# marl/l3embedding

Hardware: AMD Instinct MI355X
Metric: AVC training pairs/sec (1s audio + 224x224 frame) (higher is better)
Workload: dtype f32; 1 GPU; full cnn_L3_melspec2 AVC training step (audio+vision+fusion, fwd+bwd+Adam), batch 64 per GPU, global batch 64, fp32, inputs resident in HBM; global_batch=64, parallelism=dp1, fp32_conv=f4x4

## Files before the change

include/l3hip.h:

```cpp
#ifndef L3HIP_H
#define L3HIP_H

#include <stdint.h>

#ifdef __cplusplus
extern "C" {
#endif

#define L3_OK 0
#define L3_EINVAL (-1)
#define L3_EHIP (-2)
#define L3_ENOMEM (-3)
#define L3_ESTATE (-4)
#define L3_ECOMM (-5)

#define L3_MODEL_CNN_L3_ORIG 0
#define L3_MODEL_TINY_L3 1
#define L3_MODEL_CNN_L3_KAPREDBINPUTBN 2
#define L3_MODEL_CNN_L3_MELSPEC1 3
#define L3_MODEL_CNN_L3_MELSPEC2 4

typedef struct l3_engine l3_engine;

#define L3_DTYPE_F32 0
// ... 125 lines not shown
int l3_op_conv2d_fwd(int device, const float *x, const float *w, const float *b, float *y,
                     int n, int h, int wd, int cin, int cout, int kh, int kw, int same);
int l3_op_conv2d_bwd(int device, const float *x, const float *w, const float *dy,
                     float *dx, float *dw, float *db,
                     int n, int h, int wd, int cin, int cout, int kh, int kw, int same);
int l3_op_bn_relu_fwd(int device, const float *x, const float *gamma, const float *beta,
                      float *y, float *mean, float *var, int64_t rows, int c, int relu, int x_bf16);
int l3_op_bn_relu_bwd(int device, const float *x, const float *y, const float *dy,
                      const float *gamma, const float *beta, const float *mean, const float *var,
                      float *dx, float *dgamma, float *dbeta, int64_t rows, int c, int relu, int x_bf16);
int l3_op_bn_relu_pool2_fwd(int device, const float *x, const float *gamma, const float *beta, float *p,
                            float *mean, float *var, int n, int h, int wd, int c, int same, int relu_mode, int x_bf16);
int l3_op_bn_relu_pool2_bwd(int device, const float *x, const float *gamma, const float *beta, const float *dp,
                            float *dx, float *dgamma, float *dbeta, float *dbias, int n, int h, int wd, int c,
                            int same, int relu_mode, int x_bf16);
int l3_op_maxpool_fwd(int device, const float *x, float *y, int n, int h, int wd, int c,
                      int ph, int pw, int sh, int sw, int same);
int l3_op_maxpool_bwd(int device, const float *x, const float *dy, float *dx, int n, int h,
                      int wd, int c, int ph, int pw, int sh, int sw, int same);
int l3_op_frontend(int device, int model_type, const float *audio, int n, int db_max_scope, float *out);
int l3_op_gather_frames(int device, const float *samples, int64_t n_samples, const int64_t *table,
                        int64_t n_frames, float *frames);
int l3_op_resample(int device, const float *x, int64_t n_in, int64_t sr_orig, int64_t sr_new, const double *half_window,
                   int64_t n_window, int num_table, int64_t t0, int64_t n_out, float *y);
int l3_op_resample_clips(int device, const float *x, int64_t n_in, const int64_t *clips, int64_t n_clips, int64_t sr_new,
                         const double *half_window, int64_t n_window, int num_table, int64_t n_samples, int copy_equal,
                         float *y);
int l3_op_bn_stats_from_partials(int device, const float *part, int nblk, int c, const float *pivot, int64_t rows,
                                 float eps, float *mean, float *var);
int l3_op_conv2d_fwd_stats(int device, int dtype, const float *x, const float *w, const float *b, float *y, float *part, int *nblk,
// ... 205 lines not shown
```

l3embedding_amd/_lib.py:

```python
import ctypes as C
import os

import numpy as np

from . import _build

MODEL_IDS = {
    'cnn_L3_orig': 0,
    'tiny_L3': 1,
    'cnn_L3_kapredbinputbn': 2,
    'cnn_L3_melspec1': 3,
    'cnn_L3_melspec2': 4,
}

FAMILIES = ('conv_fwd', 'conv_dgrad', 'conv_wgrad', 'elementwise', 'frontend', 'head', 'adam')


DTYPES = {'f32': 0, 'fp32': 0, 'float32': 0, 'bf16': 1}
FP32_CONV = {'f4x4': 0, 'f2x2': 1, 'f2x2_bf16x6': 2}
DP_MOVING = {'replicas': 0, 'rank_local': 1}
OP_DTYPES = dict(DTYPES, bf16_stored=2, bf16_stored_out=3)


class L3Config(C.Structure):
# ... 89 lines not shown
    'l3_sync': (C.c_int, [C.c_void_p]),
    'l3_profile_enable': (C.c_int, [C.c_void_p, C.c_int]),
    'l3_set_tower_overlap': (C.c_int, [C.c_void_p, C.c_int]),
    'l3_profile_read_executed': (C.c_int, [C.c_void_p, C.c_int, C.POINTER(C.c_double)]),
    'l3_profile_read_bytes': (C.c_int, [C.c_void_p, C.c_int, C.POINTER(C.c_double)]),
    'l3_profile_read': (C.c_int, [C.c_void_p, C.c_int, C.POINTER(C.c_double), C.POINTER(C.c_int64),
                                  C.POINTER(C.c_double)]),
    'l3_op_conv2d_fwd': (C.c_int, [C.c_int, C.c_void_p, C.c_void_p, C.c_void_p, C.c_void_p] + [C.c_int] * 8),
    'l3_op_conv2d_fwd_dt': (C.c_int, [C.c_int, C.c_int, C.c_void_p, C.c_void_p, C.c_void_p, C.c_void_p] + [C.c_int] * 8),
    'l3_op_conv2d_bwd_dt': (C.c_int, [C.c_int, C.c_int] + [C.c_void_p] * 6 + [C.c_int] * 8),
    'l3_op_conv2d_bwd': (C.c_int, [C.c_int] + [C.c_void_p] * 6 + [C.c_int] * 8),
    'l3_op_bn_relu_fwd': (C.c_int, [C.c_int] + [C.c_void_p] * 6 + [C.c_int64, C.c_int, C.c_int, C.c_int]),
    'l3_op_bn_relu_bwd': (C.c_int, [C.c_int] + [C.c_void_p] * 10 + [C.c_int64, C.c_int, C.c_int, C.c_int]),
    'l3_op_bn_relu_pool2_fwd': (C.c_int, [C.c_int] + [C.c_void_p] * 6 + [C.c_int] * 7),
    'l3_op_bn_relu_pool2_bwd': (C.c_int, [C.c_int] + [C.c_void_p] * 8 + [C.c_int] * 7),
    'l3_op_maxpool_fwd': (C.c_int, [C.c_int, C.c_void_p, C.c_void_p] + [C.c_int] * 9),
    'l3_op_maxpool_bwd': (C.c_int, [C.c_int, C.c_void_p, C.c_void_p, C.c_void_p] + [C.c_int] * 9),
    'l3_op_frontend': (C.c_int, [C.c_int, C.c_int, C.c_void_p, C.c_int, C.c_int, C.c_void_p]),
    'l3_op_gather_frames': (C.c_int, [C.c_int, C.c_void_p, C.c_int64, C.c_void_p, C.c_int64, C.c_void_p]),
    'l3_op_resample': (C.c_int, [C.c_int, C.c_void_p, C.c_int64, C.c_int64, C.c_int64, C.c_void_p, C.c_int64, C.c_int,
                                 C.c_int64, C.c_int64, C.c_void_p]),
    'l3_op_resample_clips': (C.c_int, [C.c_int, C.c_void_p, C.c_int64, C.c_void_p, C.c_int64, C.c_int64, C.c_void_p, C.c_int64,
                                       C.c_int, C.c_int64, C.c_int, C.c_void_p]),
    'l3_op_bn_stats_from_partials': (C.c_int, [C.c_int, C.c_void_p, C.c_int, C.c_int, C.c_void_p, C.c_int64, C.c_float,
                                               C.c_void_p, C.c_void_p]),
    'l3_op_conv2d_fwd_stats': (C.c_int, [C.c_int, C.c_int] + [C.c_void_p] * 5 + [C.POINTER(C.c_int), C.c_void_p, C.c_void_p] +
                               [C.c_int] * 9),
    'l3_op_conv2d_dgrad_bn_bwd': (C.c_int, [C.c_int, C.c_int] + [C.c_void_p] * 9 + [C.POINTER(C.c_int), C.c_void_p, C.c_void_p] +
                                  [C.c_int] * 9 + [C.c_int64]),
    'l3_op_bn_relu_pool2_fwd_xwin': (C.c_int, [C.c_int] + [C.c_void_p] * 7 + [C.c_int] * 7),
# ... 627 lines not shown
                                      _ptr(var), n, h, wd, c, int(same), int(relu_mode), flags))
    return p, mean, var


def op_bn_relu_pool2_bwd(x, gamma, beta, dp, same, device=0, relu_mode=1, x_bf16=False, out_bf16=False):
    lib = load()
    x, dp = _f32(x), _f32(dp)
    n, h, wd, c = x.shape
    dx = np.empty_like(x)
    dg, db, dbias = (np.empty((c,), np.float32) for _ in range(3))
    check(lib.l3_op_bn_relu_pool2_bwd(device, _ptr(x), _ptr(_f32(gamma)), _ptr(_f32(beta)), _ptr(dp), _ptr(dx),
                                      _ptr(dg), _ptr(db), _ptr(dbias), n, h, wd, c, int(same), int(relu_mode), int(x_bf16) | (4 if out_bf16 else 0)))
    return dx, dg, db, dbias


def _pool_out(h, p, s, same):
    return -(-h // s) if same else (h - p) // s + 1


def op_maxpool_fwd(x, ph, pw, sh, sw, same, device=0):
    lib = load()
    x = _f32(x)
    n, h, wd, c = x.shape
    y = np.empty((n, _pool_out(h, ph, sh, same), _pool_out(wd, pw, sw, same), c), np.float32)
    check(lib.l3_op_maxpool_fwd(device, _ptr(x), _ptr(y), n, h, wd, c, ph, pw, sh, sw, int(same)))
    return y


def op_maxpool_bwd(x, dy, ph, pw, sh, sw, same, device=0):
    lib = load()
# ... 1044 lines not shown
```

l3embedding_amd/csrc/bn_fused.hip:

```cpp
#include "kernels.h"
#include "device_common.h"

namespace l3 {



__device__ __forceinline__ void store_quad(void* base, int64_t q, f32x4 v, int obf) {
    if (obf) {
        bf16x4 h;
        h[0] = (__bf16)v.x; h[1] = (__bf16)v.y; h[2] = (__bf16)v.z; h[3] = (__bf16)v.w;
        __builtin_nontemporal_store(h, reinterpret_cast<bf16x4*>(base) + q);
    } else {
        __builtin_nontemporal_store(v, reinterpret_cast<f32x4*>(base) + q);
    }
}

template <bool XBF>
__device__ __forceinline__ f32x4 load_quad(const void* base, int64_t q) {
    if constexpr (XBF) {
        const u32x2 r = __builtin_nontemporal_load(reinterpret_cast<const u32x2*>(base) + q);
        return f32x4{__uint_as_float(r.x << 16), __uint_as_float(r.x & 0xffff0000u), __uint_as_float(r.y << 16),
                     __uint_as_float(r.y & 0xffff0000u)};
    } else {
        return __builtin_nontemporal_load(reinterpret_cast<const f32x4*>(base) + q);
// ... 563 lines not shown
    const int nb_a = fast_blocks(work_a);
    float* part2 = dbias ? part : nullptr;
    using ApplyFn = void (*)(const void*, const void*, const f32x4*, const f32x4*, const f32x4*, const f32x4*, const f32x4*, void*,
                             float*, int64_t, Pool2Geom, int, int);
    static const ApplyFn apply_fns[8] = {
        bn_bwd_apply_fast_kernel<false, false, false>, bn_bwd_apply_fast_kernel<false, false, true>,
        bn_bwd_apply_fast_kernel<false, true, false>,  bn_bwd_apply_fast_kernel<false, true, true>,
        bn_bwd_apply_fast_kernel<true, false, false>,  bn_bwd_apply_fast_kernel<true, false, true>,
        bn_bwd_apply_fast_kernel<true, true, false>,   bn_bwd_apply_fast_kernel<true, true, true>};
    hipLaunchKernelGGL(apply_fns[variant], dim3(nb_a), dim3(FB), 0, s, xv, dyv, sc4, sh4, reinterpret_cast<const f32x4*>(cA),
                       reinterpret_cast<const f32x4*>(cB), reinterpret_cast<const f32x4*>(cC), (void*)dx, part2, n4, g, relu,
                       dx_bf16);
    if (dbias) launch_fast_final(SumFinal{dbias}, part, nb_a, C, s);
}

}
```

l3embedding_amd/csrc/elementwise.hip:

```cpp
#include <algorithm>

#include "kernels.h"

namespace l3 {

static constexpr int RED_BLOCK = 256;
static constexpr int RED_MAX_BLOCKS = 1024;
static constexpr int SMALLC_MAX = 16;

static inline int red_blocks(int64_t rows, int C) {
    int rows_per_pass = (C % 4 == 0 && C >= 4 && C <= 1024) ? (RED_BLOCK / (C / 4) > 0 ? RED_BLOCK / (C / 4) : 1) : RED_BLOCK;
    int64_t b = (rows + (int64_t)rows_per_pass * 16 - 1) / ((int64_t)rows_per_pass * 16);
    if (b < 1) b = 1;
    if (b > RED_MAX_BLOCKS) b = RED_MAX_BLOCKS;
    return (int)b;
}

size_t colreduce_scratch_floats(int64_t rows, int C) {
    const size_t a = (size_t)red_blocks(rows, C) * 2 * (size_t)(C < 4 ? 4 : C) + 64;
    const size_t b = bn_fast_ok(C) ? bn_fast_scratch_floats(C) : 0;
    return a > b ? a : b;
}

template <class F>
// ... 510 lines not shown
    int arg[4];
    const size_t base = (size_t)n * P * C + cb * 64 + cq * 4;
    gp_scan(x + base, P, C, pg, best, arg);
    gp_merge(sb, sa, pg, cq, best, arg);
    const gp4 d = *reinterpret_cast<const gp4*>(dy + (size_t)n * out_batch_stride + cb * 64 + cq * 4);
    int am[4];
#pragma unroll
    for (int e = 0; e < 4; ++e) am[e] = sa[0][cq * 4 + e];
    for (int p = pg; p < P; p += 16) {
        gp4 o;
#pragma unroll
        for (int e = 0; e < 4; ++e) o[e] = p == am[e] ? d[e] : 0.f;
        *reinterpret_cast<gp4*>(dx + base + (size_t)p * C) = o;
    }
}
static bool is_global_pool(const PoolGeom& g) {
    return g.Ho == 1 && g.Wo == 1 && g.padT == 0 && g.padL == 0 && g.ph == g.H && g.pw == g.W && g.C % 64 == 0 &&
           g.out_batch_stride % 4 == 0;
}

void maxpool_fwd(const float* x, float* y, const PoolGeom& g, hipStream_t s) {
    if (is_global_pool(g)) {
        hipLaunchKernelGGL(global_maxpool_fwd_kernel, dim3(g.N * (g.C / 64)), dim3(256), 0, s, x, y, g.H * g.W, g.C,
                           (int64_t)g.out_batch_stride);
        return;
    }
    const int64_t total = (int64_t)g.N * g.Ho * g.Wo * g.C;
    hipLaunchKernelGGL(maxpool_fwd_kernel, dim3(ew_blocks(total)), dim3(256), 0, s, x, y, g);
}
__global__ __launch_bounds__(256) void maxpool_bwd_kernel(const float* x, const float* dy, float* dx, PoolGeom g) {
    const int64_t total = (int64_t)g.N * g.Ho * g.Wo * g.C;
// ... 395 lines not shown
```

l3embedding_amd/csrc/engine.hip:

```cpp
#include <hip/hip_runtime.h>
#include "knobs.h"

#include <cmath>
#include <cstdio>
#include <cstdlib>
#include <cstring>
#include <map>
#include <string>
#include <vector>

#include "../../include/l3hip.h"
#include "comm.h"
#include "conv_path.h"
#include "kernels.h"

namespace {

using namespace l3;

static thread_local std::string g_create_error;

constexpr float BN_EPS = 1e-3f;
constexpr float BN_MOMENTUM = 0.99f;
constexpr float L2_WEIGHT = 1e-5f;
// ... 28 lines not shown
};

enum FirstWgrad { FW_NONE, FW_AUG, FW_AUG_DEFERRED };
struct ConvPlan {
    ConvStorage st;
    ConvFwdPath fwd;
    int stat_mode = 0;
    FirstWgrad aug = FW_NONE;
    ConvWgradPath wgrad;
    bool colsum = false;
    ConvDgradPath dgrad;
    int bwd_bn = -1;
    double fwd_bytes = 0.0, wg_bytes = 0.0, dg_bytes = 0.0;
};
enum BnStats { BS_PARTIALS, BS_FAST, BS_PLAIN, BS_MOVING };
enum BnBwd { BB_BY_FIRST_CONV, BB_FAST_POOLED, BB_FAST, BB_FAST_DEFERRED, BB_PLAIN };
struct BnPlan {
    BnStats stats = BS_MOVING;
    int stat_blocks = 0;
    BnBwd bwd = BB_PLAIN;
    int bwd_blocks = 0;
    double fwd_bytes = 0.0, bwd_bytes = 0.0;
};

struct Op {
    OpKind kind;
    std::string name;
    int in = 0, out = 0;
    int block = 0, bucket = 0;
    int kh = 0, kw = 0, cout = 0;
    bool same = false;
// ... 6 lines not shown
    bool fused_first = false;
    bool defer_apply = false;
    int bn_defer = -1;
    float *xaug = nullptr, *gaug = nullptr;
    ConvGeom ageom{};
    int bn_follow = -1;
    bool need_dx = true;
    int dy_to_bn = -1;
    float* xwin = nullptr;
    int p_gamma = -1, p_beta = -1, p_mmean = -1, p_mvar = -1;
    bool fused_relu = false;
    bool prerelu = false;
    int fuse_pool = -1;
    int bias_param = -1;
    bool fused_into_bn = false;
    bool bias_by_bn = false;
    float *mean = nullptr, *var = nullptr, *scale = nullptr, *shift = nullptr;
    float *biased_mean = nullptr, *biased_var = nullptr;
    PoolGeom pg{};
    ConvPlan cp{};
    BnPlan bp{};
};

struct Tower {
    std::string prefix;
    std::vector<Tensor> t;
    std::vector<Op> ops;
    int nblocks = 0;
    int emb_conv_op = -1;
    bool training = false;
// ... 464 lines not shown
                    bn.fused_first = true;
                    op.ageom = op.geom;
                    op.ageom.Cin = op.geom.Cin + 1;
                }
                break;
            }
    const int nbv = e->vis.nblocks, nba = e->aud.nblocks;
    for (auto& op : e->vis.ops) op.bucket = 1 + (nbv - 1 - op.block);
    for (auto& op : e->aud.ops) op.bucket = 1 + nbv + (nba - 1 - op.block);
    for (Tower* tw : {&e->vis, &e->aud})
        for (auto& op : tw->ops) {
            for (int pi : {op.p_kernel, op.p_bias, op.p_gamma, op.p_beta})
                if (pi >= 0) e->params[pi].bucket = op.bucket;
        }
    for (int pi : {e->p_w1, e->p_b1, e->p_w2, e->p_b2}) e->params[pi].bucket = 0;
    for (Tower* tw : {&e->vis, &e->aud})
        for (size_t i = 0; i < tw->ops.size(); ++i) {
            Op& op = tw->ops[i];
            if (op.kind != OP_BN || !bn_fast_ok(tw->t[op.in].C)) continue;
            if (i > 0 && tw->ops[i - 1].kind == OP_CONV) {
                op.bias_param = tw->ops[i - 1].p_bias;
                tw->ops[i - 1].bias_by_bn = true;
                tw->ops[i - 1].bn_follow = (int)i;
            }
            const bool pool_next = i + 2 < tw->ops.size() && tw->ops[i + 1].kind == OP_POOL &&
                                   tw->ops[i + 1].pg.ph == 2 && tw->ops[i + 1].pg.pw == 2 && tw->ops[i + 1].pg.sh == 2 &&
                                   tw->ops[i + 1].pg.sw == 2 && tw->ops[i + 1].pg.padT == 0 && tw->ops[i + 1].pg.padL == 0;
            if (op.fused_relu && pool_next) {
                op.fuse_pool = (int)i + 1;
                tw->ops[i + 1].fused_into_bn = true;
            } else if (!op.fused_relu && pool_next && i >= 2 && tw->ops[i - 1].kind == OP_RELU &&
                       tw->ops[i - 2].kind == OP_CONV) {
                op.prerelu = true;
                op.in = tw->ops[i - 2].out;
                tw->ops[i - 1].fused_into_bn = true;
                op.bias_param = tw->ops[i - 2].p_bias;
                tw->ops[i - 2].bias_by_bn = true;
                tw->ops[i - 2].bn_follow = (int)i;
                op.fuse_pool = (int)i + 1;
                tw->ops[i + 1].fused_into_bn = true;
            }
        }
    const int first_wg_fuse = knob_int("L3_FIRST_WG_FUSE", 1);
    if (first_wg_fuse)
        for (Tower* tw : {&e->vis, &e->aud})
            for (auto& cv : tw->ops) {
                if (cv.kind != OP_CONV || cv.in_bn < 0 || cv.bn_follow < 0 || !cv.bias_by_bn) continue;
                Op& bn = tw->ops[cv.bn_follow];
                if (bn.kind == OP_BN && bn.fuse_pool < 0 && !bn.prerelu && bn.in == cv.out && bn_fast_ok(cv.cout) &&
                    conv_first_wgrad_ok(cv.ageom)) {
                    bn.defer_apply = true;
                    cv.bn_defer = cv.bn_follow;
                }
            }
    const int pooled_fuse = knob_int("L3_BNBWD_FUSE_POOLED", 1);
    if (bnbwd_fuse && pooled_fuse)
        for (Tower* tw : {&e->vis, &e->aud})
            for (size_t i = 0; i < tw->ops.size(); ++i) {
                Op& cv = tw->ops[i];
                if (cv.kind != OP_CONV || !cv.need_dx || cv.dy_to_bn >= 0) continue;
                for (size_t j = 0; j < i; ++j) {
                    const Op& bn = tw->ops[j];
                    if (bn.kind == OP_BN && bn.fuse_pool >= 0 && tw->ops[bn.fuse_pool].out == cv.in && (bn.fused_relu != bn.prerelu) &&
                        bn_fast_ok(tw->t[bn.in].C))
// ... 325 lines not shown
        tw.t[0].d = ti == 0 ? e->video : nullptr;
        if (ti == 1) {
            if ((rc = dev_alloc_t(e, &tw.t[0].d, (size_t)tw.t[0].numel()))) return rc;
        }
        const int64_t concat_off = ti == 0 ? 0 : e->nv;
        for (size_t oi = 0; oi < tw.ops.size(); ++oi) {
            Op& op = tw.ops[oi];
            Tensor& y = tw.t[op.out];
            const bool last = oi + 1 == tw.ops.size();
            if (last) {
                y.d = e->h0 + concat_off;
                y.g = e->dh0 + concat_off;
                y.batch_stride = D;
                y.alias = true;
                if (op.kind == OP_POOL) op.pg.out_batch_stride = D;
            } else if ((op.kind == OP_BN && op.fuse_pool >= 0) || (op.kind == OP_RELU && op.fused_into_bn)) {
                if (op.kind == OP_BN) {
                    bool wanted = false;
                    for (size_t ci = 0; ci < tw.ops.size(); ++ci)
                        if (tw.ops[ci].kind == OP_CONV && tw.ops[ci].dy_to_bn == (int)oi) wanted = true;
                    const Tensor& pl = tw.t[tw.ops[op.fuse_pool].out];
                    if (wanted && (rc = dev_alloc_t(e, &op.xwin, t_floats(pl, tw.t[op.in].d_bf16)))) return rc;
                }
            } else {
                if ((rc = dev_alloc_t(e, &y.d, t_floats(y, y.d_bf16)))) return rc;
                if ((rc = dev_alloc_t(e, &y.g, t_floats(y, y.g_bf16)))) return rc;
            }
            const Tensor& x = tw.t[op.in];
            if (op.kind == OP_CONV) {
                if ((rc = dev_alloc_t(e, &op.wflip, (size_t)e->params[op.p_kernel].numel))) return rc;
// ... 166 lines not shown
        if (!op.need_dx) continue;
        p.dgrad = conv_resolve_dgrad(op.geom, op.dgeom, p.st, op.wino_ud != nullptr);
        p.dg_bytes = grad_bytes(y) + grad_bytes(x) + wbytes;
        Op* bn = training && op.dy_to_bn >= 0 && e->stat_max > 0 ? &tw.ops[op.dy_to_bn] : nullptr;
        if (bn != nullptr && bn->fuse_pool >= 0 && (bn->xwin == nullptr || x.batch_stride != (int64_t)x.H * x.W * x.C)) bn = nullptr;
        if (bn == nullptr) continue;
        const int blocks = conv_dgrad_bn_blocks(p.dgrad, op.dgeom, x.g_bf16, tw.t[bn->in].d_bf16);
        if (blocks < 0) continue;
        if (!fits(op, blocks, op.dgeom.Cout)) return L3_ESTATE;
        p.bwd_bn = op.dy_to_bn;
        bn->bp.bwd_blocks = blocks;
    }
    for (auto& op : tw.ops) {
        if (op.kind != OP_BN) continue;
        const Tensor &x = tw.t[op.in], &y = tw.t[op.out];
        const Tensor& out = op.fuse_pool >= 0 ? tw.t[tw.ops[op.fuse_pool].out] : y;
        BnPlan& p = op.bp;
        p.stats = !training ? BS_MOVING : p.stat_blocks > 0 ? BS_PARTIALS : op.prerelu || x.d_bf16 ? BS_FAST : BS_PLAIN;
        p.bwd = training && op.fused_first ? BB_BY_FIRST_CONV : !bn_fast_ok(x.C) ? BB_PLAIN : op.fuse_pool >= 0 ? BB_FAST_POOLED
                : defers(op) ? BB_FAST_DEFERRED : BB_FAST;
        p.fwd_bytes = (!training ? 0.0 : p.stat_blocks > 0 ? (double)p.stat_blocks * 2 * x.C * 4 : act_bytes(x)) + act_bytes(x) + act_bytes(out);
        if (p.bwd == BB_BY_FIRST_CONV) p.fwd_bytes += act_bytes(x) + (double)x.rows() * (&op + 1)->ageom.Cin * 4.0;
        if (op.fuse_pool >= 0 && training && op.xwin != nullptr) p.fwd_bytes += (double)out.numel() * (x.d_bf16 ? 2.0 : 4.0);
        p.bwd_bytes = p.bwd == BB_PLAIN ? 2.0 * (act_bytes(x) + grad_bytes(y)) + grad_bytes(x)
                                        : (p.bwd_blocks > 0 ? (double)p.bwd_blocks * 2 * x.C * 4 : act_bytes(x) + grad_bytes(out)) +
                                              (p.bwd == BB_FAST_DEFERRED ? 0.0 : act_bytes(x) + grad_bytes(out) + grad_bytes(x));
    }
    return L3_OK;
}

void tower_forward(l3_engine* e, Tower& tw) {
    const bool training = tw.training;
    for (auto& op : tw.ops) {
        Tensor& x = tw.t[op.in];
        Tensor& y = tw.t[op.out];
        switch (op.kind) {
            case OP_CONV: {
                const ConvPlan& p = op.cp;
                ConvBufs b;
                b.x = x.d, b.w = e->params[op.p_kernel].d, b.bias = e->params[op.p_bias].d, b.y = y.d;
                b.wprep = op.wflip, b.wino_u = op.wino_uf;
// ... 20 lines not shown
                        break;
                    case BS_PLAIN:
                        bn_stats(x.d, gamma, beta, op.mean, op.var, op.scale, op.shift, e->red_scratch, x.rows(), x.C, BN_EPS, e->stream);
                        break;
                    case BS_MOVING:
                        bn_scale_shift(gamma, beta, e->params[op.p_mmean].d, e->params[op.p_mvar].d, op.scale, op.shift, x.C, BN_EPS,
                                       e->stream);
                        break;
                }
                if (p.bwd == BB_BY_FIRST_CONV) bn_xhat_ones(x.d, op.mean, op.var, BN_EPS, (&op + 1)->xaug, x.rows(), x.C, e->stream);
                if (op.fuse_pool >= 0) {
                    Tensor& pl = tw.t[tw.ops[op.fuse_pool].out];
                    bn_relu_pool2_fwd(x.d, op.scale, op.shift, pl.d, x.N, x.H, x.W, x.C, pl.H, pl.W, pl.batch_stride,
                                      op.prerelu ? 2 : (op.fused_relu ? 1 : 0), e->stream, pl.d_bf16 ? 1 : 0, x.d_bf16 ? 1 : 0,
                                      training ? (void*)op.xwin : nullptr);
                } else if (y.d_bf16 || x.d_bf16) {
                    bn_apply_fast(x.d, op.scale, op.shift, y.d, x.rows(), x.C, op.fused_relu ? 1 : 0, e->stream, y.d_bf16 ? 1 : 0,
                                  x.d_bf16 ? 1 : 0);
                } else {
                    bn_apply(x.d, op.scale, op.shift, y.d, x.rows(), x.C, op.fused_relu ? 1 : 0, e->stream);
                }
                break;
            }
            case OP_RELU: {
                if (op.fused_into_bn) break;
                ProfScope ps(e, F_ELEMWISE, 0.0);
                ps.bytes(act_bytes(x) + act_bytes(y));
                relu_fwd(x.d, y.d, x.numel(), e->stream);
                break;
            }
// ... 35 lines not shown
                relu_bwd(y.d, y.g, x.g, x.numel(), e->stream);
                break;
            }
            case OP_BN: {
                const BnPlan& p = op.bp;
                if (p.bwd == BB_BY_FIRST_CONV) break;
                ProfScope ps(e, F_ELEMWISE, 0.0);
                ps.bytes(p.bwd_bytes);
                const float* mean = training ? op.mean : e->params[op.p_mmean].d;
                const float* var = training ? op.var : e->params[op.p_mvar].d;
                const float* gamma = e->params[op.p_gamma].d;
                float *dgamma = e->params[op.p_gamma].g, *dbeta = e->params[op.p_beta].g;
                if (p.bwd == BB_PLAIN) {
                    bn_bwd(x.d, y.d, y.g, gamma, mean, var, x.g, dgamma, dbeta, e->red_scratch, x.rows(), x.C, BN_EPS, op.fused_relu ? 1 : 0,
                           training ? 1 : 0, e->stream);
                    break;
                }
                const bool pooled = p.bwd == BB_FAST_POOLED, defer = p.bwd == BB_FAST_DEFERRED;
                const Tensor& dy = pooled ? tw.t[tw.ops[op.fuse_pool].out] : y;
                bn_bwd_fast(x.d, op.scale, op.shift, mean, var, gamma, dy.g, pooled ? 1 : 0, x.N, x.H, x.W, x.C, dy.H, dy.W,
                            pooled ? dy.batch_stride : (int64_t)x.H * x.W * x.C, defer ? nullptr : x.g, dgamma, dbeta,
                            defer ? nullptr : op.bias_param >= 0 ? e->params[op.bias_param].g : nullptr, e->red_scratch, BN_EPS,
                            pooled ? (op.prerelu ? 2 : 1) : (op.fused_relu ? 1 : 0), training ? 1 : 0, e->stream, x.g_bf16 ? 1 : 0,
                            x.d_bf16 ? 1 : 0, dy.g_bf16 ? 1 : 0, p.bwd_blocks > 0 ? e->stat_scratch : nullptr, p.bwd_blocks);
                break;
            }
            case OP_CONV: {
                const ConvPlan& p = op.cp;
                const float* w = e->params[op.p_kernel].d;
                if (p.aug != FW_NONE) {
// ... 1480 lines not shown
```

l3embedding_amd/csrc/kernels.h:

```cpp
#pragma once
#include <hip/hip_runtime.h>
#include <stdint.h>

#include <string>
#include <vector>

#include "host_common.h"

namespace l3 {

struct ConvGeom {
    int N, H, W, Cin;
    int Ho, Wo, Cout;
    int KH, KW, padT, padL;
    int f2x2 = 0;
    int solo = 0;
    int dynamic = 0;
    float* tail_scratch = nullptr;
    size_t tail_scratch_bytes = 0;
};
size_t conv_wino4_tail_scratch_bytes();

struct BnBwdFuse {
    const float* x;
// ... 96 lines not shown
                   float* shift, float* scratch, int64_t rows, int C, float eps, int prerelu, hipStream_t s, int x_bf16 = 0);
void bn_stats_from_partials(const float* part, int nblk, const float* pivot, const float* gamma, const float* beta,
                            float* mean, float* var, float* scale, float* shift, int64_t rows, int C, float eps,
                            int prerelu, hipStream_t s);
void bn_apply_fast(const float* x, const float* scale, const float* shift, float* y, int64_t rows, int C, int relu,
                   hipStream_t s, int out_bf16 = 0, int x_bf16 = 0);
void bn_relu_pool2_fwd(const float* x, const float* scale, const float* shift, float* p, int N, int H, int W, int C,
                       int Ho, int Wo, int64_t out_batch_stride, int mode, hipStream_t s, int out_bf16 = 0, int x_bf16 = 0,
                       void* xwin = nullptr);
void bn_bwd_fast(const float* x, const float* scale, const float* shift, const float* mean, const float* var,
                 const float* gamma, const float* dy, int pooled, int N, int H, int W, int C, int Ho, int Wo,
                 int64_t dy_batch_stride, float* dx, float* dgamma, float* dbeta, float* dbias, float* scratch,
                 float eps, int relu, int training, hipStream_t s, int dx_bf16 = 0, int x_bf16 = 0, int dy_bf16 = 0,
                 const float* ready_part = nullptr, int ready_blocks = 0);
const float* bn_bwd_fast_coeffs(const float* scratch, int C);

void relu_fwd(const float* x, float* y, int64_t n, hipStream_t s);
void relu_bwd(const float* y, const float* dy, float* dx, int64_t n, hipStream_t s);

struct PoolGeom {
    int N, H, W, C, Ho, Wo, ph, pw, sh, sw, padT, padL;
    int64_t out_batch_stride;
};
void maxpool_fwd(const float* x, float* y, const PoolGeom& g, hipStream_t s);
void maxpool_bwd(const float* x, const float* dy, float* dx, const PoolGeom& g, hipStream_t s);

void preprocess_video(const uint8_t* u8, float* out, int64_t n, hipStream_t s);
void preprocess_audio(const int16_t* pcm, float* out, int64_t n, hipStream_t s);
void labels_onehot(const int32_t* lab, float* out, int64_t n, hipStream_t s);

struct AugmentParams {
    int32_t start_x, start_y, flip, sat_first;
    float saturation, brightness;
};
constexpr int AUG_CROP = 224;
void augment_video(const uint8_t* u8, int N, int H, int W, const AugmentParams* params, uint8_t* out_u8, float* out_f32,
                   hipStream_t s);
void augment_audio(const int16_t* pcm, int N, int T, const double* u, int16_t* out_i16, float* out_f32, double* gains,
// ... 132 lines not shown
```

l3embedding_amd/csrc/ops.hip:

```cpp
#include <hip/hip_runtime.h>

#include <cstring>
#include <string>
#include <vector>

#include "../../include/l3hip.h"
#include "conv_path.h"
#include "kernels.h"
#include "knobs.h"
#include "mlp.h"
#include "vggish.h"

namespace {
using namespace l3;

struct Scope {
    DeviceBufs bufs;
    hipStream_t s = nullptr;
    bool ok = true;
    explicit Scope(int device) : ok(device_ok(device)) {}
    ~Scope() { (void)hipDeviceSynchronize(); }
    template <class T>
    T* alloc(size_t count) {
        T* p = bufs.alloc<T>(count);
// ... 282 lines not shown

int l3_op_bn_relu_pool2_fwd_xwin(int device, const float* x, const float* gamma, const float* beta, float* p, float* mean,
                                 float* var, float* xwin, int n, int h, int wd, int c, int same, int relu_mode, int x_bf16) {
    if (!xwin) return L3_EINVAL;
    return pool2_common(device, x, gamma, beta, nullptr, p, mean, var, nullptr, nullptr, nullptr, nullptr, n, h, wd, c,
                        same, relu_mode, x_bf16, xwin);
}

int l3_op_bn_relu_pool2_bwd(int device, const float* x, const float* gamma, const float* beta, const float* dp,
                            float* dx, float* dgamma, float* dbeta, float* dbias, int n, int h, int wd, int c, int same,
                            int relu_mode, int x_bf16) {
    return pool2_common(device, x, gamma, beta, dp, nullptr, nullptr, nullptr, dx, dgamma, dbeta, dbias, n, h, wd, c,
                        same, relu_mode, x_bf16);
}

int l3_op_maxpool_fwd(int device, const float* x, float* y, int n, int h, int wd, int c, int ph, int pw, int sh,
                      int sw, int same) {
    Scope sc(device);
    if (!sc.ok) return L3_EHIP;
    const PoolGeom g = make_pool(n, h, wd, c, ph, pw, sh, sw, same);
    float* d_x = sc.put(x, (size_t)n * h * wd * c);
    float* d_y = sc.alloc<float>((size_t)n * g.Ho * g.Wo * c);
    if (!sc.ok) return L3_ENOMEM;
    maxpool_fwd(d_x, d_y, g, sc.s);
    sc.get(y, d_y, (size_t)n * g.Ho * g.Wo * c);
    return sc.status();
}

int l3_op_maxpool_bwd(int device, const float* x, const float* dy, float* dx, int n, int h, int wd, int c, int ph,
                      int pw, int sh, int sw, int same) {
// ... 857 lines not shown
```

Measured before the change: 2077 pairs/s.

## Fuse final BN+ReLU with global max-pool in forward and backward

Adds fused kernels that apply BN scale/shift and ReLU while scanning for the per-channel global max and its argmax, so the last BN output tensor is never written. Backward uses the stored winning index and input value to compute the BN gradient reductions over N entries, then writes dx in a single pass. This targets the full-size intermediate activation writes and reads between the last BN and the global pool in both towers. It adds argmax scratch, a two-stage scan/merge, and tie-break logic that must match the existing max-pool semantics.

```diff
diff --git a/include/l3hip.h b/include/l3hip.h
--- a/include/l3hip.h
+++ b/include/l3hip.h
@@ -163,6 +163,11 @@
 int l3_op_bn_relu_pool2_bwd(int device, const float *x, const float *gamma, const float *beta, const float *dp,
                             float *dx, float *dgamma, float *dbeta, float *dbias, int n, int h, int wd, int c,
                             int same, int relu_mode, int x_bf16);
+int l3_op_bn_relu_gpool_fwd(int device, const float *x, const float *gamma, const float *beta, float *mean, float *var,
+                            float *p, int32_t *win, int n, int h, int wd, int c, int64_t stride, int training, int x_bf16);
+int l3_op_bn_relu_gpool_bwd(int device, const float *x, const float *gamma, const float *beta, float *mean, float *var,
+                            const float *g, float *dx, float *dgamma, float *dbeta, float *dbias, int n, int h, int wd, int c,
+                            int64_t stride, int training, int x_bf16);
 int l3_op_maxpool_fwd(int device, const float *x, float *y, int n, int h, int wd, int c,
                       int ph, int pw, int sh, int sw, int same);
 int l3_op_maxpool_bwd(int device, const float *x, const float *dy, float *dx, int n, int h,
diff --git a/l3embedding_amd/_lib.py b/l3embedding_amd/_lib.py
--- a/l3embedding_amd/_lib.py
+++ b/l3embedding_amd/_lib.py
@@ -127,6 +127,8 @@
     'l3_op_bn_relu_bwd': (C.c_int, [C.c_int] + [C.c_void_p] * 10 + [C.c_int64, C.c_int, C.c_int, C.c_int]),
     'l3_op_bn_relu_pool2_fwd': (C.c_int, [C.c_int] + [C.c_void_p] * 6 + [C.c_int] * 7),
     'l3_op_bn_relu_pool2_bwd': (C.c_int, [C.c_int] + [C.c_void_p] * 8 + [C.c_int] * 7),
+    'l3_op_bn_relu_gpool_fwd': (C.c_int, [C.c_int] + [C.c_void_p] * 7 + [C.c_int] * 4 + [C.c_int64, C.c_int, C.c_int]),
+    'l3_op_bn_relu_gpool_bwd': (C.c_int, [C.c_int] + [C.c_void_p] * 10 + [C.c_int] * 4 + [C.c_int64, C.c_int, C.c_int]),
     'l3_op_maxpool_fwd': (C.c_int, [C.c_int, C.c_void_p, C.c_void_p] + [C.c_int] * 9),
     'l3_op_maxpool_bwd': (C.c_int, [C.c_int, C.c_void_p, C.c_void_p, C.c_void_p] + [C.c_int] * 9),
     'l3_op_frontend': (C.c_int, [C.c_int, C.c_int, C.c_void_p, C.c_int, C.c_int, C.c_void_p]),
@@ -784,6 +786,40 @@
     return dx, dg, db, dbias
 
 
+def _gpool_moments(c, moving):
+    if moving is None:
+        return np.empty((c,), np.float32), np.empty((c,), np.float32), 1
+    mean, var = (np.array(_f32(m)) for m in moving)
+    assert mean.shape == var.shape == (c,)
+    return mean, var, 0
+
+
+def op_bn_relu_gpool_fwd(x, gamma, beta, device=0, moving=None, stride=None, fill=0.0, x_bf16=False):
+    lib = load()
+    x = _f32(x)
+    n, h, wd, c = x.shape
+    stride = c if stride is None else int(stride)
+    p = np.full((n, stride), fill, np.float32)
+    win = np.empty((n, c), np.int32)
+    mean, var, training = _gpool_moments(c, moving)
+    check(lib.l3_op_bn_relu_gpool_fwd(device, _ptr(x), _ptr(_f32(gamma)), _ptr(_f32(beta)), _ptr(mean), _ptr(var), _ptr(p), _ptr(win),
+                                      n, h, wd, c, stride, training, int(x_bf16)))
+    return p, win, mean, var
+
+
+def op_bn_relu_gpool_bwd(x, gamma, beta, g, device=0, moving=None, x_bf16=False, out_bf16=False):
+    lib = load()
+    x, g = _f32(x), _f32(g)
+    n, h, wd, c = x.shape
+    assert g.ndim == 2 and g.shape[0] == n
+    dx = np.empty_like(x)
+    dg, db, dbias = (np.empty((c,), np.float32) for _ in range(3))
+    mean, var, training = _gpool_moments(c, moving)
+    check(lib.l3_op_bn_relu_gpool_bwd(device, _ptr(x), _ptr(_f32(gamma)), _ptr(_f32(beta)), _ptr(mean), _ptr(var), _ptr(g), _ptr(dx),
+                                      _ptr(dg), _ptr(db), _ptr(dbias), n, h, wd, c, g.shape[1], training, int(x_bf16) | (4 if out_bf16 else 0)))
+    return dx, dg, db, dbias
+
+
 def _pool_out(h, p, s, same):
     return -(-h // s) if same else (h - p) // s + 1
 
diff --git a/l3embedding_amd/csrc/bn_fused.hip b/l3embedding_amd/csrc/bn_fused.hip
--- a/l3embedding_amd/csrc/bn_fused.hip
+++ b/l3embedding_amd/csrc/bn_fused.hip
@@ -601,4 +601,207 @@
     if (dbias) launch_fast_final(SumFinal{dbias}, part, nb_a, C, s);
 }
 
-}
+static constexpr int GP_U = 4;
+static constexpr int GP_FWD_ITERS = 16;
+
+static inline int gp_fwd_chunk(int C) { return FB / (C / 4) * GP_FWD_ITERS; }
+static inline int gp_fwd_chunks(int P, int C) { return (P + gp_fwd_chunk(C) - 1) / gp_fwd_chunk(C); }
+size_t bn_gpool_scratch_floats(int N, int P, int C) { return (size_t)N * gp_fwd_chunks(P, C) * C * 2; }
+
+__device__ __forceinline__ bool gp_wins(float av, int ai, float bv, int bi) { return bv > av || (bv == av && bi < ai); }
+
+template <bool XBF>
+__global__ __launch_bounds__(FB) void bn_relu_gpool_scan_kernel(const void* __restrict__ x, const f32x4* scale, const f32x4* shift,
+                                                               f32x4* __restrict__ pval, i32x4* __restrict__ pidx, int P, int C4,
+                                                               int chunk, int S) {
+    __shared__ f32x4 sv[FB];
+    __shared__ i32x4 si[FB];
+    const int t = threadIdx.x;
+    const int c4 = t % C4, pg = t / C4, G = FB / C4;
+    const int n = blockIdx.x / S, sc_i = blockIdx.x % S;
+    const int p0 = sc_i * chunk, p1 = min(P, p0 + chunk);
+    const f32x4 sc = scale[c4], sh = shift[c4];
+    const int64_t base = (int64_t)n * P * C4 + c4;
+    f32x4 best = {-INFINITY, -INFINITY, -INFINITY, -INFINITY};
+    i32x4 arg = {0x7fffffff, 0x7fffffff, 0x7fffffff, 0x7fffffff};
+    for (int p = p0 + pg; p < p1; p += G * GP_U) {
+        f32x4 v[GP_U];
+#pragma unroll
+        for (int u = 0; u < GP_U; ++u)
+            if (p + u * G < p1) v[u] = load_quad<XBF>(x, base + (int64_t)(p + u * G) * C4);
+#pragma unroll
+        for (int u = 0; u < GP_U; ++u)
+            if (p + u * G < p1) {
+                const f32x4 a = relu4(bn_pre(v[u], sc, sh));
+#pragma unroll
+                for (int e = 0; e < 4; ++e)
+                    if (a[e] > best[e] || arg[e] == 0x7fffffff) {
+                        best[e] = a[e];
+                        arg[e] = p + u * G;
+                    }
+            }
+    }
+    sv[t] = best;
+    si[t] = arg;
+    __syncthreads();
+    if (t < C4) {
+        for (int k = 1; k < G; ++k) {
+            const f32x4 bv = sv[k * C4 + t];
+            const i32x4 bi = si[k * C4 + t];
+#pragma unroll
+            for (int e = 0; e < 4; ++e)
+                if (gp_wins(best[e], arg[e], bv[e], bi[e])) {
+                    best[e] = bv[e];
+                    arg[e] = bi[e];
+                }
+        }
+        pval[(int64_t)blockIdx.x * C4 + c4] = best;
+        pidx[(int64_t)blockIdx.x * C4 + c4] = arg;
+    }
+}
+
+template <bool XBF>
+__global__ __launch_bounds__(FB) void bn_relu_gpool_merge_kernel(const void* __restrict__ x, const f32x4* __restrict__ pval,
+                                                                const i32x4* __restrict__ pidx, f32x4* __restrict__ out,
+                                                                i32x4* __restrict__ win, f32x4* __restrict__ xw, int N, int P,
+                                                                int C4, int S, int64_t out_bs4) {
+    const int i = blockIdx.x * FB + threadIdx.x;
+    if (i >= N * C4) return;
+    const int n = i / C4, c4 = i % C4;
+    f32x4 best = pval[(int64_t)n * S * C4 + c4];
+    i32x4 arg = pidx[(int64_t)n * S * C4 + c4];
+    constexpr int MU = 8;
+    for (int k0 = 1; k0 < S; k0 += MU) {
+        f32x4 bv[MU];
+        i32x4 bi[MU];
+#pragma unroll
+        for (int u = 0; u < MU; ++u)
+            if (k0 + u < S) {
+                bv[u] = pval[((int64_t)n * S + k0 + u) * C4 + c4];
+                bi[u] = pidx[((int64_t)n * S + k0 + u) * C4 + c4];
+            }
+#pragma unroll
+        for (int u = 0; u < MU; ++u)
+            if (k0 + u < S) {
+#pragma unroll
+                for (int e = 0; e < 4; ++e)
+                    if (gp_wins(best[e], arg[e], bv[u][e], bi[u][e])) {
+                        best[e] = bv[u][e];
+                        arg[e] = bi[u][e];
+                    }
+            }
+    }
+    out[(int64_t)n * out_bs4 + c4] = best;
+    if (win != nullptr) {
+        win[i] = arg;
+        f32x4 w;
+#pragma unroll
+        for (int e = 0; e < 4; ++e) w[e] = load_quad<XBF>(x, ((int64_t)n * P + arg[e]) * C4 + c4)[e];
+        xw[i] = w;
+    }
+}
+
+void bn_relu_gpool_fwd(const float* x, const float* scale, const float* shift, float* p, int N, int P, int C,
+                       int64_t out_batch_stride, int32_t* win, float* xw, float* scratch, hipStream_t s, int x_bf16) {
+    const int C4 = C / 4, chunk = gp_fwd_chunk(C), S = gp_fwd_chunks(P, C);
+    f32x4* pval = reinterpret_cast<f32x4*>(scratch);
+    i32x4* pidx = reinterpret_cast<i32x4*>(scratch + (size_t)N * S * C);
+    auto scan = x_bf16 ? bn_relu_gpool_scan_kernel<true> : bn_relu_gpool_scan_kernel<false>;
+    hipLaunchKernelGGL(scan, dim3(N * S), dim3(FB), 0, s, (const void*)x, reinterpret_cast<const f32x4*>(scale),
+                       reinterpret_cast<const f32x4*>(shift), pval, pidx, P, C4, chunk, S);
+    auto merge = x_bf16 ? bn_relu_gpool_merge_kernel<true> : bn_relu_gpool_merge_kernel<false>;
+    hipLaunchKernelGGL(merge, dim3((N * C4 + FB - 1) / FB), dim3(FB), 0, s, (const void*)x, (const f32x4*)pval, (const i32x4*)pidx,
+                       reinterpret_cast<f32x4*>(p), reinterpret_cast<i32x4*>(win), reinterpret_cast<f32x4*>(xw), N, P, C4, S,
+                       out_batch_stride / 4);
+}
+
+__device__ __forceinline__ f32x4 gp_gate(f32x4 g, f32x4 xwv, f32x4 sc, f32x4 sh) {
+    const f32x4 pre = bn_pre(xwv, sc, sh);
+    return f32x4{pre.x > 0.f ? g.x : 0.f, pre.y > 0.f ? g.y : 0.f, pre.z > 0.f ? g.z : 0.f, pre.w > 0.f ? g.w : 0.f};
+}
+
+__global__ __launch_bounds__(FB) void bn_relu_gpool_bwd_reduce_kernel(const f32x4* __restrict__ xw, const f32x4* __restrict__ g,
+                                                                     const f32x4* scale, const f32x4* shift, const f32x4* mean,
+                                                                     const f32x4* var, float* part, int N, int C4, int64_t g_bs4,
+                                                                     float eps) {
+    const int c4 = threadIdx.x % C4, G = FB / C4;
+    const f32x4 sc = scale[c4], sh = shift[c4], mu = mean[c4], vv = var[c4];
+    const f32x4 rs = {rsqrtf(vv.x + eps), rsqrtf(vv.y + eps), rsqrtf(vv.z + eps), rsqrtf(vv.w + eps)};
+    f32x4 a0 = {0.f, 0.f, 0.f, 0.f}, a1 = {0.f, 0.f, 0.f, 0.f};
+    for (int n = blockIdx.x * G + threadIdx.x / C4; n < N; n += gridDim.x * G) {
+        const f32x4 xv = xw[(int64_t)n * C4 + c4];
+        const f32x4 d = gp_gate(g[(int64_t)n * g_bs4 + c4], xv, sc, sh);
+        a0 += d;
+        a1 += d * ((xv - mu) * rs);
+    }
+    block_write_partials(a0, a1, part, C4);
+}
+
+template <bool XBF>
+__global__ __launch_bounds__(FB) void bn_relu_gpool_bwd_apply_kernel(const void* __restrict__ x, const f32x4* __restrict__ xw,
+                                                                    const i32x4* __restrict__ win, const f32x4* __restrict__ g,
+                                                                    const f32x4* scale, const f32x4* shift, const f32x4* cA,
+                                                                    const f32x4* cB, const f32x4* cC, void* __restrict__ dx,
+                                                                    float* part, int N, int P, int C4, int chunk, int S,
+                                                                    int64_t g_bs4, int obf) {
+    const int t = threadIdx.x;
+    const int c4 = t % C4, pg = t / C4, G = FB / C4;
+    const f32x4 sc = scale[c4], sh = shift[c4], A = cA[c4], B = cB[c4], Cc = cC[c4];
+    f32x4 a0 = {0.f, 0.f, 0.f, 0.f};
+    for (int item = blockIdx.x; item < N * S; item += gridDim.x) {
+        const int n = item / S, p0 = (item % S) * chunk, p1 = min(P, p0 + chunk);
+        const i32x4 w = win[(int64_t)n * C4 + c4];
+        const f32x4 d = gp_gate(g[(int64_t)n * g_bs4 + c4], xw[(int64_t)n * C4 + c4], sc, sh);
+        const int64_t base = (int64_t)n * P * C4 + c4;
+        for (int p = p0 + pg; p < p1; p += G * GP_U) {
+            f32x4 v[GP_U];
+#pragma unroll
+            for (int u = 0; u < GP_U; ++u)
+                if (p + u * G < p1) v[u] = load_quad<XBF>(x, base + (int64_t)(p + u * G) * C4);
+#pragma unroll
+            for (int u = 0; u < GP_U; ++u)
+                if (p + u * G < p1) {
+                    const int pu = p + u * G;
+                    const f32x4 dz = {pu == w.x ? d.x : 0.f, pu == w.y ? d.y : 0.f, pu == w.z ? d.z : 0.f, pu == w.w ? d.w : 0.f};
+                    const f32x4 o = A * dz + (B * v[u] + Cc);
+                    store_quad(dx, base + (int64_t)pu * C4, o, obf);
+                    a0 += o;
+                }
+        }
+    }
+    if (part != nullptr) block_write_partials(a0, a0, part, C4);
+}
+
+void bn_relu_gpool_bwd(const float* x, const float* xw, const int32_t* win, const float* g, const float* scale, const float* shift,
+                       const float* mean, const float* var, const float* gamma, int N, int P, int C, int64_t g_batch_stride,
+                       float* dx, float* dgamma, float* dbeta, float* dbias, float* scratch, float eps, int training, hipStream_t s,
+                       int dx_bf16, int x_bf16) {
+    const int C4 = C / 4, G = FB / C4;
+    float* part = scratch;
+    float* cA = scratch + (size_t)FAST_MAX_BLOCKS * 2 * C;
+    float* cB = cA + C;
+    float* cC = cB + C;
+    const f32x4* sc4 = reinterpret_cast<const f32x4*>(scale);
+    const f32x4* sh4 = reinterpret_cast<const f32x4*>(shift);
+    const f32x4* xw4 = reinterpret_cast<const f32x4*>(xw);
+    const f32x4* g4 = reinterpret_cast<const f32x4*>(g);
+    const int nb_r = (N + G - 1) / G < FAST_MAX_BLOCKS ? (N + G - 1) / G : FAST_MAX_BLOCKS;
+    hipLaunchKernelGGL(bn_relu_gpool_bwd_reduce_kernel, dim3(nb_r), dim3(FB), 0, s, xw4, g4, sc4, sh4, reinterpret_cast<const f32x4*>(mean),
+                       reinterpret_cast<const f32x4*>(var), part, N, C4, g_batch_stride / 4, eps);
+    launch_fast_final(BwdFinal{gamma, mean, var, dgamma, dbeta, cA, cB, cC, 1.0 / ((double)N * P), eps, training}, part, nb_r, C, s);
+    if (dx == nullptr) return;
+    int S = FAST_MAX_BLOCKS / N;
+    if (S < 1) S = 1;
+    if (S > gp_fwd_chunks(P, C)) S = gp_fwd_chunks(P, C);
+    const int chunk = ((P + S - 1) / S + G - 1) / G * G;
+    S = (P + chunk - 1) / chunk;
+    const int64_t items = (int64_t)N * S;
+    const int nb_a = (int)(items < FAST_MAX_BLOCKS ? items : FAST_MAX_BLOCKS);
+    auto apply = x_bf16 ? bn_relu_gpool_bwd_apply_kernel<true> : bn_relu_gpool_bwd_apply_kernel<false>;
+    hipLaunchKernelGGL(apply, dim3(nb_a), dim3(FB), 0, s, (const void*)x, xw4, reinterpret_cast<const i32x4*>(win), g4, sc4, sh4,
+                       reinterpret_cast<const f32x4*>(cA), reinterpret_cast<const f32x4*>(cB), reinterpret_cast<const f32x4*>(cC),
+                       (void*)dx, dbias ? part : nullptr, N, P, C4, chunk, S, g_batch_stride / 4, dx_bf16);
+    if (dbias) launch_fast_final(SumFinal{dbias}, part, nb_a, C, s);
+}
+
+}
diff --git a/l3embedding_amd/csrc/elementwise.hip b/l3embedding_amd/csrc/elementwise.hip
--- a/l3embedding_amd/csrc/elementwise.hip
+++ b/l3embedding_amd/csrc/elementwise.hip
@@ -548,7 +548,7 @@
         *reinterpret_cast<gp4*>(dx + base + (size_t)p * C) = o;
     }
 }
-static bool is_global_pool(const PoolGeom& g) {
+bool is_global_pool(const PoolGeom& g) {
     return g.Ho == 1 && g.Wo == 1 && g.padT == 0 && g.padL == 0 && g.ph == g.H && g.pw == g.W && g.C % 64 == 0 &&
            g.out_batch_stride % 4 == 0;
 }
diff --git a/l3embedding_amd/csrc/engine.hip b/l3embedding_amd/csrc/engine.hip
--- a/l3embedding_amd/csrc/engine.hip
+++ b/l3embedding_amd/csrc/engine.hip
@@ -66,7 +66,7 @@
     double fwd_bytes = 0.0, wg_bytes = 0.0, dg_bytes = 0.0;
 };
 enum BnStats { BS_PARTIALS, BS_FAST, BS_PLAIN, BS_MOVING };
-enum BnBwd { BB_BY_FIRST_CONV, BB_FAST_POOLED, BB_FAST, BB_FAST_DEFERRED, BB_PLAIN };
+enum BnBwd { BB_BY_FIRST_CONV, BB_FAST_POOLED, BB_FAST_GPOOL, BB_FAST, BB_FAST_DEFERRED, BB_PLAIN };
 struct BnPlan {
     BnStats stats = BS_MOVING;
     int stat_blocks = 0;
@@ -103,6 +103,8 @@
     int fuse_pool = -1;
     int bias_param = -1;
     bool fused_into_bn = false;
+    int gpool = -1;
+    int32_t* gwin = nullptr;
     bool bias_by_bn = false;
     float *mean = nullptr, *var = nullptr, *scale = nullptr, *shift = nullptr;
     float *biased_mean = nullptr, *biased_var = nullptr;
@@ -597,6 +599,7 @@
                 if (pi >= 0) e->params[pi].bucket = op.bucket;
         }
     for (int pi : {e->p_w1, e->p_b1, e->p_w2, e->p_b2}) e->params[pi].bucket = 0;
+    const int gpool_fuse = knob_int("L3_GPOOL_FUSE", 1);
     for (Tower* tw : {&e->vis, &e->aud})
         for (size_t i = 0; i < tw->ops.size(); ++i) {
             Op& op = tw->ops[i];
@@ -623,6 +626,11 @@
                 op.fuse_pool = (int)i + 1;
                 tw->ops[i + 1].fused_into_bn = true;
             }
+            if (gpool_fuse && op.fused_relu && !op.prerelu && i + 2 == tw->ops.size() && tw->ops[i + 1].kind == OP_POOL &&
+                is_global_pool(tw->ops[i + 1].pg) && (e->nv + e->na) % 4 == 0) {
+                op.gpool = (int)i + 1;
+                tw->ops[i + 1].fused_into_bn = true;
+            }
         }
     const int first_wg_fuse = knob_int("L3_FIRST_WG_FUSE", 1);
     if (first_wg_fuse)
@@ -630,7 +638,7 @@
             for (auto& cv : tw->ops) {
                 if (cv.kind != OP_CONV || cv.in_bn < 0 || cv.bn_follow < 0 || !cv.bias_by_bn) continue;
                 Op& bn = tw->ops[cv.bn_follow];
-                if (bn.kind == OP_BN && bn.fuse_pool < 0 && !bn.prerelu && bn.in == cv.out && bn_fast_ok(cv.cout) &&
+                if (bn.kind == OP_BN && bn.fuse_pool < 0 && bn.gpool < 0 && !bn.prerelu && bn.in == cv.out && bn_fast_ok(cv.cout) &&
                     conv_first_wgrad_ok(cv.ageom)) {
                     bn.defer_apply = true;
                     cv.bn_defer = cv.bn_follow;
@@ -986,6 +994,11 @@
                 y.batch_stride = D;
                 y.alias = true;
                 if (op.kind == OP_POOL) op.pg.out_batch_stride = D;
+            } else if (op.kind == OP_BN && op.gpool >= 0) {
+                if ((rc = dev_alloc_t(e, &op.xwin, (size_t)y.N * y.C))) return rc;
+                if ((rc = dev_alloc_t(e, &op.gwin, (size_t)y.N * y.C))) return rc;
+                const size_t r = bn_gpool_scratch_floats(y.N, y.H * y.W, y.C);
+                if (r > red_max) red_max = r;
             } else if ((op.kind == OP_BN && op.fuse_pool >= 0) || (op.kind == OP_RELU && op.fused_into_bn)) {
                 if (op.kind == OP_BN) {
                     bool wanted = false;
@@ -1182,17 +1195,19 @@
     for (auto& op : tw.ops) {
         if (op.kind != OP_BN) continue;
         const Tensor &x = tw.t[op.in], &y = tw.t[op.out];
-        const Tensor& out = op.fuse_pool >= 0 ? tw.t[tw.ops[op.fuse_pool].out] : y;
+        const Tensor& out = op.fuse_pool >= 0 ? tw.t[tw.ops[op.fuse_pool].out] : op.gpool >= 0 ? tw.t[tw.ops[op.gpool].out] : y;
         BnPlan& p = op.bp;
         p.stats = !training ? BS_MOVING : p.stat_blocks > 0 ? BS_PARTIALS : op.prerelu || x.d_bf16 ? BS_FAST : BS_PLAIN;
         p.bwd = training && op.fused_first ? BB_BY_FIRST_CONV : !bn_fast_ok(x.C) ? BB_PLAIN : op.fuse_pool >= 0 ? BB_FAST_POOLED
-                : defers(op) ? BB_FAST_DEFERRED : BB_FAST;
+                : op.gpool >= 0 ? BB_FAST_GPOOL : defers(op) ? BB_FAST_DEFERRED : BB_FAST;
         p.fwd_bytes = (!training ? 0.0 : p.stat_blocks > 0 ? (double)p.stat_blocks * 2 * x.C * 4 : act_bytes(x)) + act_bytes(x) + act_bytes(out);
         if (p.bwd == BB_BY_FIRST_CONV) p.fwd_bytes += act_bytes(x) + (double)x.rows() * (&op + 1)->ageom.Cin * 4.0;
         if (op.fuse_pool >= 0 && training && op.xwin != nullptr) p.fwd_bytes += (double)out.numel() * (x.d_bf16 ? 2.0 : 4.0);
         p.bwd_bytes = p.bwd == BB_PLAIN ? 2.0 * (act_bytes(x) + grad_bytes(y)) + grad_bytes(x)
                                         : (p.bwd_blocks > 0 ? (double)p.bwd_blocks * 2 * x.C * 4 : act_bytes(x) + grad_bytes(out)) +
                                               (p.bwd == BB_FAST_DEFERRED ? 0.0 : act_bytes(x) + grad_bytes(out) + grad_bytes(x));
+        if (op.gpool >= 0) p.fwd_bytes += 2.0 * out.numel() * 4.0;
+        if (p.bwd == BB_FAST_GPOOL) p.bwd_bytes = 5.0 * out.numel() * 4.0 + act_bytes(x) + grad_bytes(x);
     }
     return L3_OK;
 }
@@ -1243,6 +1258,10 @@
                     bn_relu_pool2_fwd(x.d, op.scale, op.shift, pl.d, x.N, x.H, x.W, x.C, pl.H, pl.W, pl.batch_stride,
                                       op.prerelu ? 2 : (op.fused_relu ? 1 : 0), e->stream, pl.d_bf16 ? 1 : 0, x.d_bf16 ? 1 : 0,
                                       training ? (void*)op.xwin : nullptr);
+                } else if (op.gpool >= 0) {
+                    Tensor& pl = tw.t[tw.ops[op.gpool].out];
+                    bn_relu_gpool_fwd(x.d, op.scale, op.shift, pl.d, x.N, x.H * x.W, x.C, pl.batch_stride, op.gwin, op.xwin, e->red_scratch,
+                                      e->stream, x.d_bf16 ? 1 : 0);
                 } else if (y.d_bf16 || x.d_bf16) {
                     bn_apply_fast(x.d, op.scale, op.shift, y.d, x.rows(), x.C, op.fused_relu ? 1 : 0, e->stream, y.d_bf16 ? 1 : 0,
                                   x.d_bf16 ? 1 : 0);
@@ -1308,6 +1327,13 @@
                 if (p.bwd == BB_PLAIN) {
                     bn_bwd(x.d, y.d, y.g, gamma, mean, var, x.g, dgamma, dbeta, e->red_scratch, x.rows(), x.C, BN_EPS, op.fused_relu ? 1 : 0,
                            training ? 1 : 0, e->stream);
+                    break;
+                }
+                if (p.bwd == BB_FAST_GPOOL) {
+                    const Tensor& pl = tw.t[tw.ops[op.gpool].out];
+                    bn_relu_gpool_bwd(x.d, op.xwin, op.gwin, pl.g, op.scale, op.shift, mean, var, gamma, x.N, x.H * x.W, x.C, pl.batch_stride,
+                                      x.g, dgamma, dbeta, op.bias_param >= 0 ? e->params[op.bias_param].g : nullptr, e->red_scratch, BN_EPS,
+                                      training ? 1 : 0, e->stream, x.g_bf16 ? 1 : 0, x.d_bf16 ? 1 : 0);
                     break;
                 }
                 const bool pooled = p.bwd == BB_FAST_POOLED, defer = p.bwd == BB_FAST_DEFERRED;
diff --git a/l3embedding_amd/csrc/kernels.h b/l3embedding_amd/csrc/kernels.h
--- a/l3embedding_amd/csrc/kernels.h
+++ b/l3embedding_amd/csrc/kernels.h
@@ -134,6 +134,13 @@
                  float eps, int relu, int training, hipStream_t s, int dx_bf16 = 0, int x_bf16 = 0, int dy_bf16 = 0,
                  const float* ready_part = nullptr, int ready_blocks = 0);
 const float* bn_bwd_fast_coeffs(const float* scratch, int C);
+size_t bn_gpool_scratch_floats(int N, int P, int C);
+void bn_relu_gpool_fwd(const float* x, const float* scale, const float* shift, float* p, int N, int P, int C,
+                       int64_t out_batch_stride, int32_t* win, float* xw, float* scratch, hipStream_t s, int x_bf16 = 0);
+void bn_relu_gpool_bwd(const float* x, const float* xw, const int32_t* win, const float* g, const float* scale, const float* shift,
+                       const float* mean, const float* var, const float* gamma, int N, int P, int C, int64_t g_batch_stride,
+                       float* dx, float* dgamma, float* dbeta, float* dbias, float* scratch, float eps, int training, hipStream_t s,
+                       int dx_bf16 = 0, int x_bf16 = 0);
 
 void relu_fwd(const float* x, float* y, int64_t n, hipStream_t s);
 void relu_bwd(const float* y, const float* dy, float* dx, int64_t n, hipStream_t s);
@@ -142,6 +149,7 @@
     int N, H, W, C, Ho, Wo, ph, pw, sh, sw, padT, padL;
     int64_t out_batch_stride;
 };
+bool is_global_pool(const PoolGeom& g);
 void maxpool_fwd(const float* x, float* y, const PoolGeom& g, hipStream_t s);
 void maxpool_bwd(const float* x, const float* dy, float* dx, const PoolGeom& g, hipStream_t s);
 
diff --git a/l3embedding_amd/csrc/ops.hip b/l3embedding_amd/csrc/ops.hip
--- a/l3embedding_amd/csrc/ops.hip
+++ b/l3embedding_amd/csrc/ops.hip
@@ -320,6 +320,79 @@
                         same, relu_mode, x_bf16);
 }
 
+static int gpool_common(int device, const float* x, const float* gamma, const float* beta, float* mean, float* var, float* p,
+                        int32_t* win, const float* g, float* dx, float* dgamma, float* dbeta, float* dbias, int n, int h, int wd,
+                        int c, int64_t stride, int training, int x_bf16) {
+    const PoolGeom pg = make_pool(n, h, wd, c, h, wd, h, wd, 0);
+    if (!bn_fast_ok(c) || !is_global_pool(pg) || stride < c || stride % 4) return L3_EINVAL;
+    Scope sc(device);
+    if (!sc.ok) return L3_EHIP;
+    const int P = h * wd;
+    const int64_t rows = (int64_t)n * P;
+    const size_t nx = (size_t)rows * c, np_ = (size_t)n * stride, nc = (size_t)n * c;
+    const bool obf = (x_bf16 & 4) != 0;
+    float* d_x = sc.put(x, nx);
+    float* d_g = sc.put(gamma, (size_t)c);
+    float* d_b = sc.put(beta, (size_t)c);
+    float *d_m = training ? sc.alloc<float>(c) : sc.put(mean, (size_t)c), *d_v = training ? sc.alloc<float>(c) : sc.put(var, (size_t)c);
+    float *d_sc = sc.alloc<float>(c), *d_sh = sc.alloc<float>(c);
+    float* d_p = sc.put(p, np_);
+    float* d_xw = sc.alloc<float>(nc);
+    int32_t* d_win = sc.alloc<int32_t>(nc);
+    size_t red = colreduce_scratch_floats(rows, c);
+    if (bn_gpool_scratch_floats(n, P, c) > red) red = bn_gpool_scratch_floats(n, P, c);
+    float* d_red = sc.alloc<float>(red);
+    if (!sc.ok) return L3_ENOMEM;
+    if (x_bf16 & 1) {
+        uint16_t* xb = sc.alloc<uint16_t>(nx);
+        if (!sc.ok) return L3_ENOMEM;
+        cast_bf16(d_x, xb, (int64_t)nx, sc.s);
+        d_x = reinterpret_cast<float*>(xb);
+    }
+    if (!training)
+        bn_scale_shift(d_g, d_b, d_m, d_v, d_sc, d_sh, c, 1e-3f, sc.s);
+    else if (x_bf16 & 1)
+        bn_stats_fast(d_x, d_g, d_b, d_m, d_v, d_sc, d_sh, d_red, rows, c, 1e-3f, 0, sc.s, 1);
+    else
+        bn_stats(d_x, d_g, d_b, d_m, d_v, d_sc, d_sh, d_red, rows, c, 1e-3f, sc.s);
+    bn_relu_gpool_fwd(d_x, d_sc, d_sh, d_p, n, P, c, stride, d_win, d_xw, d_red, sc.s, x_bf16 & 1);
+    sc.get(p, d_p, np_);
+    sc.get(win, d_win, nc);
+    if (training) {
+        sc.get(mean, d_m, (size_t)c);
+        sc.get(var, d_v, (size_t)c);
+    }
+    if (g) {
+        float* d_gr = sc.put(g, np_);
+        float* d_dx = sc.alloc<float>(nx);
+        float *d_dg = sc.alloc<float>(c), *d_db = sc.alloc<float>(c), *d_dbias = sc.alloc<float>(c);
+        if (!sc.ok) return L3_ENOMEM;
+        bn_relu_gpool_bwd(d_x, d_xw, d_win, d_gr, d_sc, d_sh, d_m, d_v, d_g, n, P, c, stride, d_dx, d_dg, d_db, d_dbias, d_red, 1e-3f,
+                          training ? 1 : 0, sc.s, obf ? 1 : 0, x_bf16 & 1);
+        sc.get_stored(dx, d_dx, nx, obf);
+        sc.get(dgamma, d_dg, (size_t)c);
+        sc.get(dbeta, d_db, (size_t)c);
+        sc.get(dbias, d_dbias, (size_t)c);
+    }
+    return sc.status();
+}
+
+int l3_op_bn_relu_gpool_fwd(int device, const float* x, const float* gamma, const float* beta, float* mean, float* var, float* p,
+                            int32_t* win, int n, int h, int wd, int c, int64_t stride, int training, int x_bf16) {
+    if (!p || !mean || !var) return L3_EINVAL;
+    return gpool_common(device, x, gamma, beta, mean, var, p, win, nullptr, nullptr, nullptr, nullptr, nullptr, n, h, wd, c, stride,
+                        training, x_bf16);
+}
+
+int l3_op_bn_relu_gpool_bwd(int device, const float* x, const float* gamma, const float* beta, float* mean, float* var,
+                            const float* g, float* dx, float* dgamma, float* dbeta, float* dbias, int n, int h, int wd, int c,
+                            int64_t stride, int training, int x_bf16) {
+    if (!g || !mean || !var) return L3_EINVAL;
+    std::vector<float> p((size_t)n * (stride > 0 ? stride : 0));
+    return gpool_common(device, x, gamma, beta, mean, var, p.data(), nullptr, g, dx, dgamma, dbeta, dbias, n, h, wd, c, stride,
+                        training, x_bf16);
+}
+
 int l3_op_maxpool_fwd(int device, const float* x, float* y, int n, int h, int wd, int c, int ph, int pw, int sh,
                       int sw, int same) {
     Scope sc(device);
```

Result: no change. 2093 pairs/s, median of 6 (+0.8%).
